# shubhamchandak94/Spring

Hardware: AMD Instinct MI355X
Metric: Mreads/s through reorder stage (higher is better)
Workload: dtype u64; 1 GPU; 100000000 x 150 bp single-end synthetic reads per GPU (uniform genome 600000000 bp, 25x coverage, 1.0% substitutions, 50% reverse-complemented), inputs resident in HBM as .dna records; reads_per_gpu=100000000, read_len=150, chains=65536, num_thr=8, parallelism=single GPU, unmatched=13958636, singletons=12720853, rounds=1984, chain_groups=2

## Files before the change

### include/spring_reorder.h

```cpp
#ifndef SPRING_REORDER_H_
#define SPRING_REORDER_H_

#include <stddef.h>
#include <stdint.h>

#ifdef __cplusplus
extern "C" {
#endif

#define SPRING_REORDER_E_ARG (-1)
#define SPRING_REORDER_E_IO (-2)
#define SPRING_REORDER_E_HIP (-3)
#define SPRING_REORDER_E_STATE (-4)

typedef struct spring_reorder_ctx spring_reorder_ctx;

typedef struct {
  int32_t device;
  uint32_t num_chains;
  int32_t num_thr;
  int32_t collect_stats;
  int32_t time_search;
  int32_t force_literal_update;
  int32_t rounds_per_sync;
// ... 12 lines not shown
  int32_t table_mode;
  int32_t plan0[6];
  int32_t plan1[6];
  int32_t long_min;
  int32_t long_blocks;
  int32_t debug;
  int32_t long_split;
  int32_t entry_flags;
  int32_t out_writers;
  int32_t alternatives;
  int32_t phases;
  int32_t known_absent;
  int32_t sort_prefix_bits;
  int32_t dict_build_mode;
  int32_t strand_filter;
} spring_reorder_opts;

typedef struct {
  uint64_t n_reads, n_matched, n_single, unmatched;
  uint64_t probes, keyok, cands, hits, iterations, rounds, lost;
  uint64_t numkeys[2], dict_numreads[2];
  double ms_unpack, ms_dict, ms_chains, ms_finalize, ms_total;
  double ms_search_kernel;
  uint64_t search_launches;
  uint64_t device_bytes;
  double ms_exchange, ms_resolve_mark;
  uint64_t chains;
  uint64_t deep_pool;
  uint64_t long_searches;
  uint64_t table_minz;
  uint64_t table_marked_lines;
  uint64_t long_splits;
  uint64_t alternatives;
  uint64_t phases;
  double ms_search_busy;
  uint64_t sort_prefix_bits;
  uint64_t sort_repaired_runs;
  uint64_t sort_full_sorts;
  uint64_t sort_long_runs;
  uint64_t sort_list_overflows;
  uint64_t dict_build_path;
  uint64_t strand_filter;
  uint64_t strand_filter_dropped;
} spring_reorder_stats;

void spring_reorder_default_opts(spring_reorder_opts *o);
const char *spring_reorder_last_error(void);
void spring_reorder_trim_pool(void);

int spring_reorder_run(const char *temp_dir, uint32_t max_readlen, int32_t num_thr, int32_t paired_end,
                       uint32_t num_reads_clean_0, uint32_t num_reads_clean_1,
                       const spring_reorder_opts *opts );

int spring_reorder_create(spring_reorder_ctx **ctx, const spring_reorder_opts *opts);
void spring_reorder_destroy(spring_reorder_ctx *ctx);

int spring_reorder_load_dna(spring_reorder_ctx *ctx, const uint8_t *dna, size_t nbytes, uint32_t n,
                            uint32_t max_readlen);

int spring_reorder_load_dna_device(spring_reorder_ctx *ctx, const void *d_dna, size_t nbytes, uint32_t n,
                                   uint32_t max_readlen, int32_t fixed_len);

int spring_reorder_build_dict(spring_reorder_ctx *ctx);

int spring_reorder_run_chains(spring_reorder_ctx *ctx);
int spring_reorder_auto_chains(spring_reorder_ctx *ctx, uint32_t *chains, int32_t *deep);

typedef struct {
  uint32_t num_reads[2], num_reads_clean[2], num_reads_N[2];
  uint32_t max_readlen;
  uint32_t pad;
  double ms_device;
} spring_fastq_info;
int spring_reorder_load_fastq(spring_reorder_ctx *ctx, const uint8_t *fastq_1, size_t nbytes_1, const uint8_t *fastq_2,
                              size_t nbytes_2 , spring_fastq_info *info);
int spring_reorder_fastq_N(spring_reorder_ctx *ctx, int32_t which, uint8_t *n_dna, size_t cap, size_t *nbytes,
                           uint32_t *order_N, uint32_t *count);

// ... 62 lines not shown
```

### spring_amd/_lib.py

```python
import ctypes as C
import os

HERE = os.path.dirname(os.path.abspath(__file__))
LIB_PATH = os.environ.get("SPRING_AMD_LIB") or os.path.join(HERE, "lib", "libspring_reorder_hip.so")

EXPORTS = [
    "spring_reorder_default_opts", "spring_reorder_last_error", "spring_reorder_trim_pool", "spring_reorder_run", "spring_reorder_create",
    "spring_reorder_destroy", "spring_reorder_load_dna", "spring_reorder_load_dna_device",
    "spring_reorder_build_dict", "spring_reorder_run_chains", "spring_reorder_auto_chains", "spring_reorder_finalize",
    "spring_reorder_mg_begin", "spring_reorder_mg_search", "spring_reorder_mg_slice", "spring_reorder_mg_slices",
    "spring_reorder_mg_apply",
    "spring_reorder_mg_end", "spring_reorder_mg_exchange_virtual", "spring_reorder_debug_check_seed_state",
    "spring_mg_rccl_unique_id", "spring_mg_comm_create_rccl", "spring_mg_comm_create_host", "spring_mg_comm_destroy",
    "spring_reorder_mg_run",
    "spring_reorder_get_stats", "spring_reorder_download", "spring_reorder_tid_split", "spring_reorder_emit_dna",
    "spring_reorder_dict_lookup", "spring_reorder_download_reads", "spring_synth_dna_bytes",
    "spring_reorder_load_fastq", "spring_reorder_fastq_N",
    "spring_order_invert_se", "spring_order_invert_pe", "spring_order_correct", "spring_order_pe_encode",
    "spring_fastq_reorder",
    "spring_synth_dna_host", "spring_synth_genome_host", "spring_synth_dna_device", "spring_reorder_load_synth", "spring_reorder_download_dna",
    "spring_encoder_create", "spring_encoder_destroy", "spring_encoder_set_split_tables", "spring_encoder_encode_reorder", "spring_encoder_download",
    "spring_encoder_download_seq_packed", "spring_encoder_get_info", "spring_reorder_encode_run", "spring_encoder_encode_host", "spring_encoder_run",
]

STREAMS_EXPORTS = [
    "spring_streams_create", "spring_streams_destroy", "spring_streams_from_encoder", "spring_streams_from_host",
    "spring_streams_download", "spring_streams_get_info", "spring_streams_run",
]
STREAMS_NUM = 9

DECODE_EXPORTS = [
# ... 13 lines not shown
    "spring_fastq_out_write", "spring_fastq_out_get_info",
]


class Opts(C.Structure):
    _fields_ = [("device", C.c_int32), ("num_chains", C.c_uint32), ("num_thr", C.c_int32),
                ("collect_stats", C.c_int32), ("time_search", C.c_int32), ("force_literal_update", C.c_int32),
                ("rounds_per_sync", C.c_int32), ("long_budget", C.c_int32),
                ("first_shifts", C.c_int32), ("seed_wide", C.c_int32), ("tab_scale", C.c_int32),
                ("search_wpb", C.c_int32), ("dbg_search_lds", C.c_int32), ("dbg_apply_lds", C.c_int32),
                ("fused", C.c_int32), ("deep_bins", C.c_int32),
                ("num_devices", C.c_int32), ("devices", C.c_int32 * 8), ("mg_host_transport", C.c_int32),
                ("table_mode", C.c_int32), ("plan0", C.c_int32 * 6), ("plan1", C.c_int32 * 6), ("long_min", C.c_int32),
                ("long_blocks", C.c_int32), ("debug", C.c_int32), ("long_split", C.c_int32), ("entry_flags", C.c_int32),
                ("out_writers", C.c_int32), ("alternatives", C.c_int32), ("phases", C.c_int32), ("known_absent", C.c_int32),
                ("sort_prefix_bits", C.c_int32), ("dict_build_mode", C.c_int32), ("strand_filter", C.c_int32)]


class FastqInfo(C.Structure):
    _fields_ = [("num_reads", C.c_uint32 * 2), ("num_reads_clean", C.c_uint32 * 2), ("num_reads_N", C.c_uint32 * 2),
                ("max_readlen", C.c_uint32), ("pad", C.c_uint32), ("ms_device", C.c_double)]


class EncoderInfo(C.Structure):
    _fields_ = ([(k, C.c_uint64) for k in ("n_aligned", "n_total", "seq_len", "noise_bytes", "n_noisepos",
                                           "unaligned_bytes", "len_unaligned", "num_contigs")]
                + [(k, C.c_uint32) for k in ("matched_s", "matched_N", "align_passes", "max_bin")]
                + [("ms_device", C.c_double), ("ms_phase", C.c_double * 8)])

    def asdict(self):
        d = {}
# ... 64 lines not shown


class Stats(C.Structure):
    _fields_ = ([(k, C.c_uint64) for k in ("n_reads", "n_matched", "n_single", "unmatched", "probes", "keyok",
                                          "cands", "hits", "iterations", "rounds", "lost")]
                + [("numkeys", C.c_uint64 * 2), ("dict_numreads", C.c_uint64 * 2)]
                + [(k, C.c_double) for k in ("ms_unpack", "ms_dict", "ms_chains", "ms_finalize", "ms_total",
                                             "ms_search_kernel")]
                + [("search_launches", C.c_uint64), ("device_bytes", C.c_uint64),
                   ("ms_exchange", C.c_double), ("ms_resolve_mark", C.c_double), ("chains", C.c_uint64),
                   ("deep_pool", C.c_uint64), ("long_searches", C.c_uint64),
                   ("table_minz", C.c_uint64), ("table_marked_lines", C.c_uint64), ("long_splits", C.c_uint64), ("alternatives", C.c_uint64), ("phases", C.c_uint64),
                   ("ms_search_busy", C.c_double),
                   ("sort_prefix_bits", C.c_uint64), ("sort_repaired_runs", C.c_uint64), ("sort_full_sorts", C.c_uint64),
                   ("sort_long_runs", C.c_uint64), ("sort_list_overflows", C.c_uint64), ("dict_build_path", C.c_uint64),
                   ("strand_filter", C.c_uint64), ("strand_filter_dropped", C.c_uint64)])

    def asdict(self):
        d = {}
        for k, _ in self._fields_:
            v = getattr(self, k)
            d[k] = list(v) if hasattr(v, "__len__") else v
        return d


MG_ALLGATHER_FN = C.CFUNCTYPE(C.c_int, C.c_void_p, C.c_size_t, C.c_size_t, C.c_size_t, C.c_void_p)

_lib = None


def lib():
# ... 27 lines not shown
                                           C.POINTER(C.c_uint32)]
    L.spring_reorder_debug_check_seed_state.argtypes = [vp, C.c_int32, C.POINTER(C.c_uint64)]
    L.spring_reorder_mg_apply.argtypes = [vp, C.c_int32, C.POINTER(C.c_uint32)]
    L.spring_reorder_mg_end.argtypes = [vp]
    L.spring_reorder_mg_exchange_virtual.argtypes = [C.POINTER(vp), C.c_uint32]
    L.spring_mg_rccl_unique_id.argtypes = [vp]
    L.spring_mg_comm_create_rccl.argtypes = [C.POINTER(vp), C.c_int32, vp, C.c_uint32, C.c_uint32]
    L.spring_mg_comm_create_host.argtypes = [C.POINTER(vp), MG_ALLGATHER_FN, vp, C.c_uint32, C.c_uint32]
    L.spring_mg_comm_destroy.argtypes = [vp]
    L.spring_mg_comm_destroy.restype = None
    L.spring_reorder_mg_run.argtypes = [vp, vp, C.c_uint32]
    L.spring_reorder_get_stats.argtypes = [vp, C.POINTER(Stats)]
    L.spring_reorder_download.argtypes = [vp] + [vp] * 8
    L.spring_reorder_tid_split.argtypes = [vp, vp, vp]
    L.spring_reorder_emit_dna.argtypes = [vp, C.c_int32, u8p, C.c_size_t, C.POINTER(C.c_size_t)]
    L.spring_reorder_dict_lookup.argtypes = [vp, C.c_int32, vp, C.c_uint32, vp, vp, C.c_size_t]
    L.spring_reorder_download_reads.argtypes = [vp, vp, vp]
    L.spring_reorder_load_fastq.argtypes = [vp, vp, C.c_size_t, vp, C.c_size_t, C.POINTER(FastqInfo)]
    L.spring_reorder_fastq_N.argtypes = [vp, C.c_int32, vp, C.c_size_t, C.POINTER(C.c_size_t), vp, C.POINTER(C.c_uint32)]
    L.spring_order_invert_se.argtypes = [vp, C.c_uint32, vp, C.POINTER(C.c_double)]
    L.spring_order_invert_pe.argtypes = [vp, C.c_uint32, vp, C.POINTER(C.c_double)]
    L.spring_fastq_reorder.argtypes = [u8p, C.c_size_t, vp, C.c_uint32, u8p, C.c_size_t, C.POINTER(C.c_size_t),
                                       C.POINTER(C.c_double)]
    L.spring_order_pe_encode.argtypes = [vp, C.c_uint32, vp, C.POINTER(C.c_double)]
    L.spring_order_correct.argtypes = [vp, C.c_uint64, vp, C.c_uint32, C.c_uint32, C.POINTER(C.c_double)]
    L.spring_synth_dna_bytes.restype = C.c_size_t
    L.spring_synth_dna_bytes.argtypes = [C.c_uint32, C.c_uint32]
    L.spring_synth_dna_host.argtypes = [u8p, C.c_uint32, C.c_uint32, C.c_uint64, C.c_uint64, C.c_uint32]
    L.spring_synth_genome_host.argtypes = [u8p, C.c_uint64, C.c_uint64, C.c_uint32]
    L.spring_synth_dna_device.argtypes = [vp, C.c_uint32, C.c_uint32, C.c_uint64, C.c_uint64, C.c_uint32]
# ... 80 lines not shown
```

### spring_amd/csrc/dict_build.h

```cpp
#ifndef SPRING_DICT_BUILD_H_
#define SPRING_DICT_BUILD_H_

#include "reorder_device.h"

namespace sr {

bool launch_unpack_keys(hipStream_t st, const uint8_t *dna, uint32_t n, int L, int W, int S, uint32_t rec_fixed,
                        uint64_t *reads, uint16_t *lens, uint32_t *bad_len, int dstart0, int dend0, int dstart1, int dend1,
                        uint64_t *keys0, uint32_t *vals0, uint64_t *keys1, uint32_t *vals1);

constexpr int TAB_WRITE_LG = 10;
inline int tab_write_lg(int bshift) { return 64 - bshift < TAB_WRITE_LG ? 64 - bshift : TAB_WRITE_LG; }
inline uint32_t tab_write_blocks(int bshift) { return (uint32_t)(1ull << (64 - bshift - tab_write_lg(bshift))); }
void launch_tab_partition(hipStream_t st, const uint64_t *h0, uint32_t nk0, const uint64_t *h1, uint32_t nk1, int bshift,
                          uint32_t *part);
constexpr uint32_t TAB_OVF_SLOTS = 8;
void launch_tab_write(hipStream_t st, const uint64_t *h0, uint32_t nk0, const uint64_t *h1, uint32_t nk1,
                      const uint32_t *part, DictBuild d0, DictBuild d1, uint4 *fpt, int bshift, uint32_t *ovf,
                      uint32_t *ovf_blk, uint32_t *ovf_cnt);
void launch_tab_overflow_blocks(hipStream_t st, const uint64_t *h0, uint32_t nk0, const uint64_t *h1, DictBuild d0,
                                DictBuild d1, uint32_t *fpt, int bshift, const uint32_t *ovf_blk, const uint32_t *ovf_cnt);
void launch_tab_overflow_pairs(hipStream_t st, const uint64_t *h0, uint32_t nk0, const uint64_t *h1, DictBuild d0,
                               DictBuild d1, uint32_t *fpt, int bshift, const uint32_t *ovf, uint32_t novf);

constexpr uint32_t PRES_DROP_CTRS = 1024;
void launch_pres_insert(hipStream_t st, const uint64_t *h0, uint32_t nk0, const uint64_t *h1, uint32_t nk1, int wl, uint32_t *pres,
                        int lgb, uint32_t *drops);

}

#endif
```

### spring_amd/csrc/dict_build.hip

```cpp
#include <hip/hip_runtime.h>

#include "dict_build.h"
#include "strand_filter.h"

namespace sr {

__device__ __forceinline__ uint64_t db_mix64(uint64_t x) {
  x ^= x >> 33; x *= 0xff51afd7ed558ccdull; x ^= x >> 33; x *= 0xc4ceb9fe1a85ec53ull; x ^= x >> 33;
  return x;
}
__device__ __forceinline__ uint64_t db_unmix64(uint64_t x) {
  x ^= x >> 33; x *= 0x9cb4b2f8129337dbull; x ^= x >> 33; x *= 0x4f74430c22a54005ull; x ^= x >> 33;
  return x;
}
__device__ __forceinline__ uint32_t db_fp30_of(uint64_t h) {
  const uint32_t f = (uint32_t)h & 0x3fffffffu;
  return f == 0u ? 1u : f == 0x3fffffffu ? 0x3ffffffeu : f;
}

__global__ __launch_bounds__(256) void k_unpack_fixed_keys(const uint8_t *__restrict__ dna, uint32_t n, int L, int W, int lgS,
                                                           uint32_t rec, uint64_t *__restrict__ reads,
                                                           uint16_t *__restrict__ lens, uint32_t *__restrict__ bad_len,
                                                           int dstart0, int klen0, int dstart1, int klen1,
                                                           uint64_t *__restrict__ keys0, uint32_t *__restrict__ vals0,
// ... 285 lines not shown
        placed = true;
      }
    }
    if (!placed) atomicAdd(&s_drop, 1u);
  }
  __syncthreads();
  if (threadIdx.x == 0 && s_drop) atomicAdd(drops + (blockIdx.x & (PRES_DROP_CTRS - 1u)), s_drop);
}
void launch_pres_insert(hipStream_t st, const uint64_t *h0, uint32_t nk0, const uint64_t *h1, uint32_t nk1, int wl, uint32_t *pres,
                        int lgb, uint32_t *drops) {
  const uint64_t nt = (uint64_t)nk0 + nk1;
  if (!nt) return;
  hipLaunchKernelGGL(k_pres_insert, dim3((unsigned)((nt + 255) / 256)), dim3(256), 0, st, h0, nk0, h1, nk1, wl, pres, lgb, drops);
}

}
```

### spring_amd/csrc/reorder_pipeline.cpp

```cpp
#include <hip/hip_runtime.h>
#include <dlfcn.h>

#include <algorithm>
#include <system_error>
#include <thread>
#include <memory>
#include <atomic>
#include <chrono>
#include <cstdarg>
#include <cstdio>
#include <cstdlib>
#include <cstring>
#include <map>
#include <mutex>
#include <new>
#include <stdexcept>
#include <string>
#include <unordered_map>
#include <vector>
#include <zlib.h>

#include "reorder_device.h"
#include "dict_build.h"
#include "reorder_internal.h"
// ... 310 lines not shown
    for (auto &kv : p.free_blocks) { (void)hipFree(kv.second); p.sizes.erase(kv.second); }
    p.free_blocks.clear();
    p.cached = 0;
  }
}

int spring_reorder_create(spring_reorder_ctx **out, const spring_reorder_opts *opts) {
  if (!out) return fail(SPRING_REORDER_E_ARG, "ctx is NULL");
  spring_reorder_opts o;
  if (opts) o = *opts; else spring_reorder_default_opts(&o);
  if (o.num_thr <= 0) return fail(SPRING_REORDER_E_ARG, "num_thr must be >= 1");
  if (o.sort_prefix_bits < 0 || o.sort_prefix_bits > 64)
    return fail(SPRING_REORDER_E_ARG, "sort_prefix_bits: 0 (library's choice) or 1 .. 64 bits of the key hash (64 = the full sort)");
  if (o.dict_build_mode < 0 || o.dict_build_mode > 1)
    return fail(SPRING_REORDER_E_ARG, "dict_build_mode: 0 (library's choice) or 1 (key pass, memset, merge and insert passes)");
  if (o.strand_filter < -1 || o.strand_filter > 32)
    return fail(SPRING_REORDER_E_ARG, "strand_filter: 0 (library's choice), -1 (off) or 1 .. 32 (on, at most 2^n buckets)");
  int ndev = 0;
  HIPCHK(hipGetDeviceCount(&ndev));
  if (ndev <= 0) return fail(SPRING_REORDER_E_HIP, "no HIP device");
  int dev = o.device;
  if (dev < 0) HIPCHK(hipGetDevice(&dev));
  if (dev >= ndev) return fail(SPRING_REORDER_E_ARG, "device %d out of range (%d devices)", dev, ndev);
  HIPCHK(hipSetDevice(dev));
  spring_reorder_ctx *ctx = new spring_reorder_ctx();
  ctx->o = o;
  ctx->dev = dev;
  memset(&ctx->P, 0, sizeof(ctx->P));
  memset(&ctx->stats, 0, sizeof(ctx->stats));
  HIPCHK(hipStreamCreateWithFlags(&ctx->st, hipStreamNonBlocking));
// ... 808 lines not shown
  }
  const uint64_t nk0 = ctx->dict[0].numkeys, nk1 = ctx->dict[1].numkeys, nm = nk0 + nk1;
  const int tab_scale = ctx->o.tab_scale > 0 ? ctx->o.tab_scale : 2;
  const uint64_t nb = std::max<uint64_t>(8, pow2ceil(std::max<uint64_t>(2, (nm * 10 + 15) / 16)) * (uint64_t)pow2ceil(tab_scale));
  ctx->bshift = 64;
  for (uint64_t v = nb; v > 1; v >>= 1) ctx->bshift--;
  ctx->minz = (ctx->dict[0].end - ctx->dict[0].start + 1 == MINZ_WL && ctx->L <= 192 && ctx->o.table_mode == 2) ? 1 : 0;
  ctx->lshift = 32 - (64 - ctx->bshift - 2);
  if (ctx->lshift < 1) return fail(SPRING_REORDER_E_ARG, "build_dict: table too large for minimizer addressing");
  ctx->stats.table_minz = ctx->minz; ctx->stats.table_marked_lines = 0;
  DMALLOC(ctx->fpt, nb * 32);
  const bool one_pass = nm && !ctx->minz && ctx->o.dict_build_mode != 1;
  if (!one_pass) HIPCHK(hipMemsetAsync(ctx->fpt, 0, nb * 32, st));
  uint32_t *const tab_words = reinterpret_cast<uint32_t *>(ctx->fpt);
  DBG_T("alloc+memset tab");
  if (one_pass) {
    if (nm >= 0xffffffffull) return fail(SPRING_REORDER_E_ARG, "build_dict: %llu keys exceed the 32-bit index space of the table build", (unsigned long long)nm);
    ctx->stats.dict_build_path |= 2;
    ctx->marked_lines = 0;
    DictBuild db[2];
    for (int l = 0; l < 2; l++) {
      DictDev &d = ctx->dict[l];
      db[l].ustart = ustart[l]; db[l].ucount = ucount[l]; db[l].ids = d.ids; db[l].urec = d.urec;
      db[l].deep = d.deep; db[l].ndeep = d.d_ndeep;
    }
    uint32_t *d_part = nullptr, *d_ovf = nullptr, *d_ovf_blk = nullptr, *d_ovf_cnt = nullptr, novf = 0;
    const size_t nblk = tab_write_blocks(ctx->bshift);
    DMALLOC(d_part, 2 * (nblk + 1) * 4);
    DMALLOC(d_ovf_blk, nblk * TAB_OVF_SLOTS * 4);
    DMALLOC(d_ovf_cnt, nblk * 4);
    DMALLOC(d_ovf, ((size_t)nm + 1) * 4);
    HIPCHK(hipMemsetAsync(d_ovf, 0, 4, st));
    launch_tab_partition(st, uhash[0], (uint32_t)nk0, uhash[1], (uint32_t)nk1, ctx->bshift, d_part);
    launch_tab_write(st, uhash[0], (uint32_t)nk0, uhash[1], (uint32_t)nk1, d_part, db[0], db[1], ctx->fpt, ctx->bshift, d_ovf,
                     d_ovf_blk, d_ovf_cnt);
    launch_tab_overflow_blocks(st, uhash[0], (uint32_t)nk0, uhash[1], db[0], db[1], tab_words, ctx->bshift, d_ovf_blk, d_ovf_cnt);
    HIPCHK(hipGetLastError());
    HIPCHK(hipMemcpyAsync(&novf, d_ovf, 4, hipMemcpyDeviceToHost, st));
    uint32_t nd[2][3] = {{0, 0, 0}, {0, 0, 0}};
    for (int l = 0; l < 2; l++)
      HIPCHK(hipMemcpyAsync(nd[l], ctx->dict[l].d_ndeep, 12, hipMemcpyDeviceToHost, st));
    HIPCHK(hipStreamSynchronize(st));
    DBG_T("table write");
    launch_tab_overflow_pairs(st, uhash[0], (uint32_t)nk0, uhash[1], db[0], db[1], tab_words, ctx->bshift, d_ovf, novf);
    HIPCHK(hipGetLastError());
    for (int l = 0; l < 2; l++) { ctx->dict[l].ndeep = nd[l][0]; ctx->dict[l].big_reads = nd[l][1]; ctx->dict[l].mid_reads = nd[l][2]; }
    if (dbg) {
      fprintf(stderr, "[dict] %u of %llu pairs past the %u overflow slots of their workgroup\n", novf, (unsigned long long)nm, TAB_OVF_SLOTS);
      fprintf(stderr, "[dict] reads %u + %u, keys %u + %u, bins >= %u: %u + %u, reads in bins >= %u: %u + %u, >= %u: %u + %u\n",
              ctx->dict[0].numreads, ctx->dict[1].numreads, ctx->dict[0].numkeys, ctx->dict[1].numkeys, DEEP_BIN, nd[0][0], nd[1][0],
              MID_BIN, nd[0][2], nd[1][2], BIG_BIN, nd[0][1], nd[1][1]);
    }
// ... 46 lines not shown
      DMALLOC(tp_in, nm * 8); DMALLOC(tp_out, nm * 8);
      launch_minz_prepare(st, h_in, v_in, nm, db[0], db[1], ctx->lshift, bk_in, tp_in);
      DBG_T("minz prepare");
      const unsigned end_bit = (unsigned)(64 - ctx->bshift);
      size_t tb = 0;
      HIPCHK(sort_pairs_u32_u64(st, nullptr, tb, bk_in, bk_out, tp_in, tp_out, nm, end_bit));
      DMALLOC(d_tmp2, tb);
      HIPCHK(sort_pairs_u32_u64(st, d_tmp2, tb, bk_in, bk_out, tp_in, tp_out, nm, end_bit));
      DBG_T("minz sort");
      DMALLOC(d_marked, 16);
      HIPCHK(hipMemsetAsync(d_marked, 0, 4, st));
      launch_tab_insert_minz(st, bk_out, tp_out, nm, tab_words, ctx->bshift, d_marked);
      HIPCHK(hipMemcpyAsync(&ctx->marked_lines, d_marked, 4, hipMemcpyDeviceToHost, st));
    }
    HIPCHK(hipGetLastError());
    uint32_t nd[2][3] = {{0, 0, 0}, {0, 0, 0}};
    for (int l = 0; l < 2; l++)
      HIPCHK(hipMemcpyAsync(nd[l], ctx->dict[l].d_ndeep, 12, hipMemcpyDeviceToHost, st));
    HIPCHK(hipStreamSynchronize(st));
    for (int l = 0; l < 2; l++) { ctx->dict[l].ndeep = nd[l][0]; ctx->dict[l].big_reads = nd[l][1]; ctx->dict[l].mid_reads = nd[l][2]; }
    if (dbg) fprintf(stderr, "[dict] reads %u + %u, keys %u + %u, bins >= %u: %u + %u, reads in bins >= %u: %u + %u, >= %u: %u + %u\n",
                     ctx->dict[0].numreads, ctx->dict[1].numreads, ctx->dict[0].numkeys, ctx->dict[1].numkeys, DEEP_BIN, nd[0][0], nd[1][0],
                     MID_BIN, nd[0][2], nd[1][2], BIG_BIN, nd[0][1], nd[1][1]);
    ctx->stats.table_marked_lines = ctx->marked_lines;
    DBG_T("insert");
    ctx->dfree(mv0); ctx->dfree(mh); ctx->dfree(mv); ctx->dfree(d_tmp);
    ctx->dfree(bk_in); ctx->dfree(bk_out); ctx->dfree(tp_in); ctx->dfree(tp_out); ctx->dfree(d_tmp2); ctx->dfree(d_marked); ctx->dfree(d_ovf);
  }
  ctx->pres = nullptr; ctx->pres_lgb = 0;
  ctx->stats.strand_filter = 0; ctx->stats.strand_filter_dropped = 0;
  int lgb = 0;
  if (nm && nm < 0xffffffffull && strand_filter_wanted(ctx)) {
    while (lgb < 32 && (1ull << lgb) < nm) lgb++;
    if (ctx->o.strand_filter > 0) lgb = std::min(lgb, ctx->o.strand_filter);
    if (ctx->dmalloc((void **)&ctx->pres, (size_t)16 << lgb)) {
      (void)hipGetLastError();
      ctx->pres = nullptr;
      if (dbg) fprintf(stderr, "[dict] presence table: no room for 2^%d buckets, running without\n", lgb);
    }
  }
  if (ctx->pres) {
    uint32_t *d_drops = nullptr;
    std::vector<uint32_t> h_drops(PRES_DROP_CTRS);
    DMALLOC(d_drops, PRES_DROP_CTRS * 4);
    HIPCHK(hipMemsetAsync(ctx->pres, 0, (size_t)16 << lgb, st));
    HIPCHK(hipMemsetAsync(d_drops, 0, PRES_DROP_CTRS * 4, st));
    launch_pres_insert(st, uhash[0], (uint32_t)nk0, uhash[1], (uint32_t)nk1, ctx->dict[0].end - ctx->dict[0].start + 1,
                       reinterpret_cast<uint32_t *>(ctx->pres), lgb, d_drops);
    HIPCHK(hipGetLastError());
    HIPCHK(hipMemcpyAsync(h_drops.data(), d_drops, PRES_DROP_CTRS * 4, hipMemcpyDeviceToHost, st));
    HIPCHK(hipStreamSynchronize(st));
    for (uint32_t v : h_drops) ctx->stats.strand_filter_dropped += v;
    ctx->pres_lgb = lgb;
    ctx->dfree(d_drops);
    if (dbg) fprintf(stderr, "[dict] presence table: 2^%d buckets, %llu of %llu keys dropped\n", lgb,
                     (unsigned long long)ctx->stats.strand_filter_dropped, (unsigned long long)nm);
    DBG_T("presence table");
  }
  for (int l = 0; l < 2; l++) { ctx->dfree(uhash[l]); ctx->dfree(ustart[l]); ctx->dfree(ucount[l]); }
  DBG_T("free temps");
  HIPCHK(hipEventRecord(ctx->ev[3], st));
  ctx->stage = ST_DICT;
  return 0;
}

int spring_reorder_dict_lookup(spring_reorder_ctx *ctx, int32_t which, const uint64_t *keys, uint32_t nkeys,
                               uint32_t *bin_size, uint32_t *bin_ids, size_t ids_cap) {
  if (!ctx || ctx->stage < ST_DICT) return fail(SPRING_REORDER_E_STATE, "dict_lookup: build_dict first");
  if (which < 0 || which > 1) return fail(SPRING_REORDER_E_ARG, "which must be 0 or 1");
  HIPCHK(hipSetDevice(ctx->dev));
  DictDev &d = ctx->dict[which];
  uint64_t *dk = nullptr;
  uint32_t *ds = nullptr, *dc = nullptr;
  DMALLOC(dk, (size_t)nkeys * 8);
  DMALLOC(ds, (size_t)nkeys * 4);
  DMALLOC(dc, (size_t)nkeys * 4);
  std::vector<uint32_t> hs(nkeys), hc(nkeys), hids(d.numreads);
// ... 1370 lines not shown
```

### spring_amd/csrc/strand_filter.h

```cpp
#ifndef SPRING_STRAND_FILTER_H_
#define SPRING_STRAND_FILTER_H_

#include <stdint.h>

#if defined(__HIPCC__) || defined(__CUDACC__)
#define SF_FN __host__ __device__ inline
#else
#define SF_FN inline
#endif

namespace sf {

SF_FN uint64_t mix64(uint64_t x) {
  x ^= x >> 33; x *= 0xff51afd7ed558ccdull; x ^= x >> 33; x *= 0xc4ceb9fe1a85ec53ull; x ^= x >> 33;
  return x;
}
SF_FN uint64_t brev64(uint64_t x) {
  x = ((x >> 1) & 0x5555555555555555ull) | ((x & 0x5555555555555555ull) << 1);
  x = ((x >> 2) & 0x3333333333333333ull) | ((x & 0x3333333333333333ull) << 2);
  x = ((x >> 4) & 0x0f0f0f0f0f0f0f0full) | ((x & 0x0f0f0f0f0f0f0f0full) << 4);
  x = ((x >> 8) & 0x00ff00ff00ff00ffull) | ((x & 0x00ff00ff00ff00ffull) << 8);
  x = ((x >> 16) & 0x0000ffff0000ffffull) | ((x & 0x0000ffff0000ffffull) << 16);
  return (x >> 32) | (x << 32);
}
// ... 22 lines not shown
  return r < w ? r : w;
}
SF_FN uint32_t flags_of_key(uint64_t w, int wl, int l) {
  uint32_t f;
  (void)canon_and_flags(w, wl, l, f);
  return f;
}
SF_FN uint32_t absent_of(uint32_t s0, uint32_t s1, uint32_t s2, uint32_t s3, uint32_t fp) {
  const uint32_t f0 = (s0 >> 4) == fp ? s0 : 0u, f1 = (s1 >> 4) == fp ? s1 : 0u, f2 = (s2 >> 4) == fp ? s2 : 0u,
                 f3 = (s3 >> 4) == fp ? s3 : 0u;
  const uint32_t hit = f0 | f1 | f2 | f3;
  return s3 != 0u ? 0u : ~hit & 15u;
}
SF_FN uint32_t to_window_frame(uint32_t a, bool swapped) { return swapped ? ((a >> 2) | (a << 2)) & 15u : a; }

}

#endif
```

### spring_amd/reorder.py

```python
import ctypes as C
from dataclasses import dataclass

import numpy as np

from . import _lib


class ReorderError(RuntimeError):
    """Raised where the reference throws std::runtime_error (call_template_functions.cpp:60)."""


@dataclass
class ReorderOpts:
    device: int = -1
    num_chains: int = 0
    num_thr: int = 1
    collect_stats: bool = False
    time_search: bool = False
    force_literal_update: bool = False
    rounds_per_sync: int = 0
    first_shifts: int = 0
    seed_wide: int = 0
    tab_scale: int = 0
    search_wpb: int = 0
# ... 7 lines not shown
    plan0: tuple = ()
    plan1: tuple = ()
    long_min: int = 0
    long_blocks: int = 0
    entry_flags: int = 0
    long_split: int = 0
    debug: bool = False
    out_writers: int = 0
    alternatives: int = 0
    table_mode: int = 0
    phases: int = 0
    known_absent: int = 0
    sort_prefix_bits: int = 0
    dict_build_mode: int = 0
    strand_filter: int = 0

    def to_c(self):
        o = _lib.Opts()
        _lib.lib().spring_reorder_default_opts(C.byref(o))
        o.device, o.num_chains, o.num_thr = self.device, self.num_chains, self.num_thr
        o.collect_stats, o.time_search = int(self.collect_stats), int(self.time_search)
        o.force_literal_update, o.rounds_per_sync = int(self.force_literal_update), self.rounds_per_sync
        o.first_shifts, o.seed_wide, o.tab_scale = self.first_shifts, self.seed_wide, self.tab_scale
        o.search_wpb, o.dbg_search_lds, o.dbg_apply_lds = self.search_wpb, self.dbg_search_lds, self.dbg_apply_lds
        o.fused, o.deep_bins = self.fused, self.deep_bins
        o.long_budget = self.long_budget
        if len(self.devices) > 8:
            raise ValueError("at most 8 devices")
        o.table_mode = self.table_mode
        for i, v in enumerate(tuple(self.plan0)[:6]):
            o.plan0[i] = int(v)
        for i, v in enumerate(tuple(self.plan1)[:6]):
            o.plan1[i] = int(v)
        o.long_min, o.long_blocks, o.debug = self.long_min, self.long_blocks, int(self.debug)
        o.long_split, o.entry_flags = self.long_split, self.entry_flags
        o.out_writers = self.out_writers
        o.alternatives = self.alternatives
        o.phases = self.phases
        o.known_absent = self.known_absent
        o.sort_prefix_bits = self.sort_prefix_bits
        o.dict_build_mode = self.dict_build_mode
        o.strand_filter = self.strand_filter
        o.num_devices = len(self.devices)
        for i, d in enumerate(self.devices):
            o.devices[i] = d
        o.mg_host_transport = int(self.mg_host_transport)
        return o


def _chk(rc):
    if rc != 0:
        raise ReorderError("%s (code %d)" % (_lib.lib().spring_reorder_last_error().decode(), rc))


class ReorderStage:

    def __init__(self, opts: ReorderOpts = None):
# ... 104 lines not shown
    def emit_dna(self, tid: int) -> bytes:
        nb = C.c_size_t()
        _chk(self._L.spring_reorder_emit_dna(self._h, tid, None, 0, C.byref(nb)))
        buf = np.zeros(max(nb.value, 1), np.uint8)
        _chk(self._L.spring_reorder_emit_dna(self._h, tid, buf.ctypes.data, nb.value, C.byref(nb)))
        return buf[:nb.value].tobytes()

    def dict_lookup(self, which, keys):
        keys = np.ascontiguousarray(keys, dtype=np.uint64)
        sizes = np.zeros(max(len(keys), 1), np.uint32)
        ids = np.zeros(max(self.n, 1) * 2, np.uint32)
        _chk(self._L.spring_reorder_dict_lookup(self._h, which, keys.ctypes.data, len(keys), sizes.ctypes.data,
                                                ids.ctypes.data, len(ids)))
        return sizes[:len(keys)], ids

    def download_reads(self):
        W = (2 * self.max_readlen - 1) // 64 + 1
        limbs = np.zeros((max(self.n, 1), W), np.uint64)
        ln = np.zeros(max(self.n, 1), np.uint16)
        _chk(self._L.spring_reorder_download_reads(self._h, limbs.ctypes.data, ln.ctypes.data))
        return limbs[:self.n], ln[:self.n]

    def download_dna(self) -> bytes:
        nb = self._L.spring_synth_dna_bytes(self.n, self.max_readlen)
        buf = np.zeros(max(nb, 1), np.uint8)
        _chk(self._L.spring_reorder_download_dna(self._h, buf.ctypes.data, nb))
        p = 0
        for _ in range(self.n):
            p += 2 + ((int(buf[p]) | (int(buf[p + 1]) << 8)) + 3) // 4
        return buf[:p].tobytes()
# ... 45 lines not shown
```

Baseline: 362.9 Mreads/s.

## Build presence table by streaming sorted key ranges through LDS-resident blocks

Replaces the global-atomic insert pass for the strand-filter presence table with a blocked build. Keys whose reverse complement is canonical are first compacted into a side list and radix-sorted by bucket prefix. Each workgroup then binary-searches its slice of the already-sorted hash arrays and assembles one table block in LDS with shared atomics before writing it out. This removes the full-table memset and the scattered global atomics and drops one stream synchronize. In exchange it adds a compaction kernel, a rocprim sort, a partition kernel and extra scratch memory, and it falls back to the old pass when allocation fails.

```diff
diff --git a/include/spring_reorder.h b/include/spring_reorder.h
--- a/include/spring_reorder.h
+++ b/include/spring_reorder.h
@@ -50,6 +50,7 @@
   int32_t sort_prefix_bits;
   int32_t dict_build_mode;
   int32_t strand_filter;
+  int32_t pres_build;
 } spring_reorder_opts;
 
 typedef struct {
@@ -78,6 +79,7 @@
   uint64_t dict_build_path;
   uint64_t strand_filter;
   uint64_t strand_filter_dropped;
+  uint64_t pres_build;
 } spring_reorder_stats;
 
 void spring_reorder_default_opts(spring_reorder_opts *o);
@@ -98,6 +100,8 @@
                                    uint32_t max_readlen, int32_t fixed_len);
 
 int spring_reorder_build_dict(spring_reorder_ctx *ctx);
+
+int spring_reorder_pres_table(spring_reorder_ctx *ctx, uint32_t *out, size_t cap_words, int32_t *lgb);
 
 int spring_reorder_run_chains(spring_reorder_ctx *ctx);
 int spring_reorder_auto_chains(spring_reorder_ctx *ctx, uint32_t *chains, int32_t *deep);
diff --git a/spring_amd/_lib.py b/spring_amd/_lib.py
--- a/spring_amd/_lib.py
+++ b/spring_amd/_lib.py
@@ -14,7 +14,7 @@
     "spring_mg_rccl_unique_id", "spring_mg_comm_create_rccl", "spring_mg_comm_create_host", "spring_mg_comm_destroy",
     "spring_reorder_mg_run",
     "spring_reorder_get_stats", "spring_reorder_download", "spring_reorder_tid_split", "spring_reorder_emit_dna",
-    "spring_reorder_dict_lookup", "spring_reorder_download_reads", "spring_synth_dna_bytes",
+    "spring_reorder_dict_lookup", "spring_reorder_pres_table", "spring_reorder_download_reads", "spring_synth_dna_bytes",
     "spring_reorder_load_fastq", "spring_reorder_fastq_N",
     "spring_order_invert_se", "spring_order_invert_pe", "spring_order_correct", "spring_order_pe_encode",
     "spring_fastq_reorder",
@@ -58,7 +58,8 @@
                 ("table_mode", C.c_int32), ("plan0", C.c_int32 * 6), ("plan1", C.c_int32 * 6), ("long_min", C.c_int32),
                 ("long_blocks", C.c_int32), ("debug", C.c_int32), ("long_split", C.c_int32), ("entry_flags", C.c_int32),
                 ("out_writers", C.c_int32), ("alternatives", C.c_int32), ("phases", C.c_int32), ("known_absent", C.c_int32),
-                ("sort_prefix_bits", C.c_int32), ("dict_build_mode", C.c_int32), ("strand_filter", C.c_int32)]
+                ("sort_prefix_bits", C.c_int32), ("dict_build_mode", C.c_int32), ("strand_filter", C.c_int32),
+                ("pres_build", C.c_int32)]
 
 
 class FastqInfo(C.Structure):
@@ -153,7 +154,7 @@
                    ("ms_search_busy", C.c_double),
                    ("sort_prefix_bits", C.c_uint64), ("sort_repaired_runs", C.c_uint64), ("sort_full_sorts", C.c_uint64),
                    ("sort_long_runs", C.c_uint64), ("sort_list_overflows", C.c_uint64), ("dict_build_path", C.c_uint64),
-                   ("strand_filter", C.c_uint64), ("strand_filter_dropped", C.c_uint64)])
+                   ("strand_filter", C.c_uint64), ("strand_filter_dropped", C.c_uint64), ("pres_build", C.c_uint64)])
 
     def asdict(self):
         d = {}
@@ -211,6 +212,7 @@
     L.spring_reorder_download.argtypes = [vp] + [vp] * 8
     L.spring_reorder_tid_split.argtypes = [vp, vp, vp]
     L.spring_reorder_emit_dna.argtypes = [vp, C.c_int32, u8p, C.c_size_t, C.POINTER(C.c_size_t)]
+    L.spring_reorder_pres_table.argtypes = [vp, vp, C.c_size_t, C.POINTER(C.c_int32)]
     L.spring_reorder_dict_lookup.argtypes = [vp, C.c_int32, vp, C.c_uint32, vp, vp, C.c_size_t]
     L.spring_reorder_download_reads.argtypes = [vp, vp, vp]
     L.spring_reorder_load_fastq.argtypes = [vp, vp, C.c_size_t, vp, C.c_size_t, C.POINTER(FastqInfo)]
diff --git a/spring_amd/csrc/dict_build.h b/spring_amd/csrc/dict_build.h
--- a/spring_amd/csrc/dict_build.h
+++ b/spring_amd/csrc/dict_build.h
@@ -27,6 +27,15 @@
 void launch_pres_insert(hipStream_t st, const uint64_t *h0, uint32_t nk0, const uint64_t *h1, uint32_t nk1, int wl, uint32_t *pres,
                         int lgb, uint32_t *drops);
 
+constexpr int PRES_WRITE_LG = 12;
+inline int pres_write_lg(int lgb) { return lgb < PRES_WRITE_LG ? lgb : PRES_WRITE_LG; }
+inline uint32_t pres_write_blocks(int lgb) { return 1u << (lgb - pres_write_lg(lgb)); }
+void launch_pres_swapped(hipStream_t st, const uint64_t *h0, uint32_t nk0, const uint64_t *h1, uint32_t nk1, int wl, uint64_t *ent,
+                         uint32_t *n_ent);
+hipError_t pres_sort_entries(hipStream_t st, void *tmp, size_t &tmp_bytes, const uint64_t *in, uint64_t *out, uint32_t n, int lgb);
+void launch_pres_write(hipStream_t st, const uint64_t *h0, uint32_t nk0, const uint64_t *h1, uint32_t nk1, const uint64_t *ent,
+                       uint32_t nsw, int wl, uint32_t *part, uint4 *pres, int lgb, uint32_t *drops);
+
 }
 
 #endif
diff --git a/spring_amd/csrc/dict_build.hip b/spring_amd/csrc/dict_build.hip
--- a/spring_amd/csrc/dict_build.hip
+++ b/spring_amd/csrc/dict_build.hip
@@ -1,4 +1,8 @@
 #include <hip/hip_runtime.h>
+
+#include <cstring>
+
+#include <rocprim/rocprim.hpp>
 
 #include "dict_build.h"
 #include "strand_filter.h"
@@ -323,4 +327,120 @@
   hipLaunchKernelGGL(k_pres_insert, dim3((unsigned)((nt + 255) / 256)), dim3(256), 0, st, h0, nk0, h1, nk1, wl, pres, lgb, drops);
 }
 
-}
+constexpr uint32_t PRES_SWAP_KEYS = 1024;
+__global__ __launch_bounds__(256) void k_pres_swapped(const uint64_t *__restrict__ h0, uint32_t nk0, const uint64_t *__restrict__ h1,
+                                                      uint32_t nk1, int wl, uint64_t *__restrict__ ent, uint32_t *__restrict__ n_ent) {
+  __shared__ uint64_t s_ent[PRES_SWAP_KEYS];
+  __shared__ uint32_t s_n, s_base;
+  if (threadIdx.x == 0) s_n = 0u;
+  __syncthreads();
+  const uint64_t nt = (uint64_t)nk0 + nk1, base = (uint64_t)blockIdx.x * PRES_SWAP_KEYS;
+  for (uint32_t j = 0; j < PRES_SWAP_KEYS / 256u; j++) {
+    const uint64_t t = base + j * 256u + threadIdx.x;
+    if (t >= nt) break;
+    const int l = t >= nk0 ? 1 : 0;
+    const uint64_t key = db_unmix64(l ? h1[t - nk0] : h0[t]), r = sf::rc_window(key, wl);
+    if (r < key) s_ent[atomicAdd(&s_n, 1u)] = sf::pack_entry(sf::mix64(r), l);
+  }
+  __syncthreads();
+  const uint32_t n = s_n;
+  if (threadIdx.x == 0 && n) s_base = atomicAdd(n_ent, n);
+  __syncthreads();
+  if (n) {
+    uint64_t *__restrict__ out = ent + s_base;
+    for (uint32_t k = threadIdx.x; k < n; k += 256u) out[k] = s_ent[k];
+  }
+}
+
+__global__ void k_pres_partition(const uint64_t *__restrict__ h0, uint32_t nk0, const uint64_t *__restrict__ h1, uint32_t nk1,
+                                 const uint64_t *__restrict__ ent, uint32_t nsw, int lgb, int lg_blk, uint32_t nblk,
+                                 uint32_t *__restrict__ part) {
+  const uint64_t t = (uint64_t)blockIdx.x * blockDim.x + threadIdx.x, per = (uint64_t)nblk + 1;
+  if (t >= 3ull * per) return;
+  const uint32_t a = (uint32_t)(t / per), j = (uint32_t)(t % per);
+  const uint64_t *__restrict__ h = a == 0 ? h0 : a == 1 ? h1 : ent;
+  const uint32_t nk = a == 0 ? nk0 : a == 1 ? nk1 : nsw;
+  uint32_t lo = 0, hi = nk;
+  if (j == nblk) {
+    lo = nk;
+  } else {
+    while (lo < hi) {
+      const uint32_t mid = lo + (hi - lo) / 2;
+      if (sf::block_of(h[mid], lgb, lg_blk) < j) lo = mid + 1; else hi = mid;
+    }
+  }
+  part[t] = lo;
+}
+
+constexpr uint32_t PRES_WRITE_THREADS = 512;
+__global__ __launch_bounds__(PRES_WRITE_THREADS) void k_pres_write(const uint64_t *__restrict__ h0, const uint64_t *__restrict__ h1,
+                                                                   const uint64_t *__restrict__ ent,
+                                                                   const uint32_t *__restrict__ part, uint32_t nblk, int wl,
+                                                                   uint4 *__restrict__ pres, int lgb, int lg_blk,
+                                                                   uint32_t *__restrict__ drops) {
+  __shared__ uint4 img4[1u << PRES_WRITE_LG];
+  uint32_t *img = reinterpret_cast<uint32_t *>(img4);
+  const uint32_t nbk = sf::block_buckets(lgb, lg_blk), bmask = nbk - 1u, blk = blockIdx.x;
+  for (uint32_t k = threadIdx.x; k < nbk; k += PRES_WRITE_THREADS) img4[k] = make_uint4(0u, 0u, 0u, 0u);
+  __syncthreads();
+  uint32_t ndrop = 0;
+  auto enter = [&](uint64_t hc, uint32_t flags) {
+    const uint32_t fp = sf::fp_of(hc), word = (fp << 4) | flags;
+    uint32_t *bk = img + 4u * (sf::bucket_of(hc, lgb) & bmask);
+    for (int sl = 0; sl < 4; sl++) {
+      const uint32_t old = atomicCAS(bk + sl, 0u, word);
+      if (old == 0u) return;
+      if ((old >> 4) == fp) {
+        if ((old & flags) != flags) atomicOr(bk + sl, flags);
+        return;
+      }
+    }
+    ndrop++;
+  };
+  const uint64_t per = (uint64_t)nblk + 1;
+  for (int l = 0; l < 2; l++) {
+    const uint64_t *__restrict__ h = l ? h1 : h0;
+    const uint64_t e = part[l * per + blk + 1];
+    for (uint64_t i = (uint64_t)part[l * per + blk] + threadIdx.x; i < e; i += PRES_WRITE_THREADS) {
+      const uint64_t hh = h[i], key = db_unmix64(hh);
+      uint32_t flags;
+      if (sf::canon_and_flags(key, wl, l, flags) != key) continue;
+      enter(hh, flags);
+    }
+  }
+  {
+    const uint64_t e = part[2 * per + blk + 1];
+    for (uint64_t i = (uint64_t)part[2 * per + blk] + threadIdx.x; i < e; i += PRES_WRITE_THREADS) {
+      const uint64_t x = ent[i];
+      enter(x, 4u << sf::entry_dict(x));
+    }
+  }
+  __syncthreads();
+  uint4 *__restrict__ out = pres + (uint64_t)blk * nbk;
+  for (uint32_t k = threadIdx.x; k < nbk; k += PRES_WRITE_THREADS) out[k] = img4[k];
+  if (ndrop) atomicAdd(drops + (blk & (PRES_DROP_CTRS - 1u)), ndrop);
+}
+
+void launch_pres_swapped(hipStream_t st, const uint64_t *h0, uint32_t nk0, const uint64_t *h1, uint32_t nk1, int wl, uint64_t *ent,
+                         uint32_t *n_ent) {
+  const uint64_t nt = (uint64_t)nk0 + nk1;
+  if (!nt) return;
+  hipLaunchKernelGGL(k_pres_swapped, dim3((unsigned)((nt + PRES_SWAP_KEYS - 1) / PRES_SWAP_KEYS)), dim3(256), 0, st, h0, nk0, h1,
+                     nk1, wl, ent, n_ent);
+}
+hipError_t pres_sort_entries(hipStream_t st, void *tmp, size_t &tmp_bytes, const uint64_t *in, uint64_t *out, uint32_t n, int lgb) {
+  const unsigned begin_bit = (unsigned)(64 - lgb + pres_write_lg(lgb));
+  return rocprim::radix_sort_keys<rocprim::radix_sort_config<rocprim::default_config, rocprim::default_config, rocprim::default_config, 0>>(
+      tmp, tmp_bytes, in, out, (size_t)n, begin_bit, 64u, st);
+}
+void launch_pres_write(hipStream_t st, const uint64_t *h0, uint32_t nk0, const uint64_t *h1, uint32_t nk1, const uint64_t *ent,
+                       uint32_t nsw, int wl, uint32_t *part, uint4 *pres, int lgb, uint32_t *drops) {
+  const int lg_blk = pres_write_lg(lgb);
+  const uint32_t nblk = sf::blocks_of(lgb, lg_blk);
+  const uint64_t nt = 3ull * ((uint64_t)nblk + 1);
+  hipLaunchKernelGGL(k_pres_partition, dim3((unsigned)((nt + 255) / 256)), dim3(256), 0, st, h0, nk0, h1, nk1, ent, nsw, lgb, lg_blk,
+                     nblk, part);
+  hipLaunchKernelGGL(k_pres_write, dim3(nblk), dim3(PRES_WRITE_THREADS), 0, st, h0, h1, ent, part, nblk, wl, pres, lgb, lg_blk, drops);
+}
+
+}
diff --git a/spring_amd/csrc/reorder_pipeline.cpp b/spring_amd/csrc/reorder_pipeline.cpp
--- a/spring_amd/csrc/reorder_pipeline.cpp
+++ b/spring_amd/csrc/reorder_pipeline.cpp
@@ -348,6 +348,8 @@
     return fail(SPRING_REORDER_E_ARG, "sort_prefix_bits: 0 (library's choice) or 1 .. 64 bits of the key hash (64 = the full sort)");
   if (o.dict_build_mode < 0 || o.dict_build_mode > 1)
     return fail(SPRING_REORDER_E_ARG, "dict_build_mode: 0 (library's choice) or 1 (key pass, memset, merge and insert passes)");
+  if (o.pres_build < 0 || o.pres_build > 2)
+    return fail(SPRING_REORDER_E_ARG, "pres_build: 0 (library's choice), 1 (insert pass) or 2 (streamed build)");
   if (o.strand_filter < -1 || o.strand_filter > 32)
     return fail(SPRING_REORDER_E_ARG, "strand_filter: 0 (library's choice), -1 (off) or 1 .. 32 (on, at most 2^n buckets)");
   int ndev = 0;
@@ -1186,6 +1188,31 @@
   if (!one_pass) HIPCHK(hipMemsetAsync(ctx->fpt, 0, nb * 32, st));
   uint32_t *const tab_words = reinterpret_cast<uint32_t *>(ctx->fpt);
   DBG_T("alloc+memset tab");
+  const bool pres_wanted = nm && nm < 0xffffffffull && strand_filter_wanted(ctx);
+  int lgb = 0;
+  if (pres_wanted) {
+    while (lgb < 32 && (1ull << lgb) < nm) lgb++;
+    if (ctx->o.strand_filter > 0) lgb = std::min(lgb, ctx->o.strand_filter);
+  }
+  bool pres_stream = pres_wanted && ctx->o.pres_build != 1 &&
+                     (ctx->o.pres_build == 2 || nm / pres_write_blocks(lgb) <= (1ull << 20));
+  uint64_t *d_ent = nullptr;
+  uint32_t *d_nent = nullptr, nsw = 0;
+  if (pres_stream && (ctx->dmalloc((void **)&d_ent, (size_t)nm * 8) || ctx->dmalloc((void **)&d_nent, 16))) {
+    (void)hipGetLastError();
+    ctx->dfree(d_ent); ctx->dfree(d_nent); d_ent = nullptr; d_nent = nullptr;
+    pres_stream = false;
+    if (dbg) fprintf(stderr, "[dict] presence table: no room for the streamed build's entries, insert pass\n");
+  }
+  const int pres_wl = ctx->dict[0].end - ctx->dict[0].start + 1;
+  auto pres_swapped_pass = [&]() -> int {
+    if (!pres_stream) return 0;
+    HIPCHK(hipMemsetAsync(d_nent, 0, 4, st));
+    launch_pres_swapped(st, uhash[0], (uint32_t)nk0, uhash[1], (uint32_t)nk1, pres_wl, d_ent, d_nent);
+    HIPCHK(hipGetLastError());
+    HIPCHK(hipMemcpyAsync(&nsw, d_nent, 4, hipMemcpyDeviceToHost, st));
+    return 0;
+  };
   if (one_pass) {
     if (nm >= 0xffffffffull) return fail(SPRING_REORDER_E_ARG, "build_dict: %llu keys exceed the 32-bit index space of the table build", (unsigned long long)nm);
     ctx->stats.dict_build_path |= 2;
@@ -1208,6 +1235,7 @@
                      d_ovf_blk, d_ovf_cnt);
     launch_tab_overflow_blocks(st, uhash[0], (uint32_t)nk0, uhash[1], db[0], db[1], tab_words, ctx->bshift, d_ovf_blk, d_ovf_cnt);
     HIPCHK(hipGetLastError());
+    if (int r = pres_swapped_pass()) return r;
     HIPCHK(hipMemcpyAsync(&novf, d_ovf, 4, hipMemcpyDeviceToHost, st));
     uint32_t nd[2][3] = {{0, 0, 0}, {0, 0, 0}};
     for (int l = 0; l < 2; l++)
@@ -1284,6 +1312,7 @@
       HIPCHK(hipMemcpyAsync(&ctx->marked_lines, d_marked, 4, hipMemcpyDeviceToHost, st));
     }
     HIPCHK(hipGetLastError());
+    if (int r = pres_swapped_pass()) return r;
     uint32_t nd[2][3] = {{0, 0, 0}, {0, 0, 0}};
     for (int l = 0; l < 2; l++)
       HIPCHK(hipMemcpyAsync(nd[l], ctx->dict[l].d_ndeep, 12, hipMemcpyDeviceToHost, st));
@@ -1298,11 +1327,12 @@
     ctx->dfree(bk_in); ctx->dfree(bk_out); ctx->dfree(tp_in); ctx->dfree(tp_out); ctx->dfree(d_tmp2); ctx->dfree(d_marked); ctx->dfree(d_ovf);
   }
   ctx->pres = nullptr; ctx->pres_lgb = 0;
-  ctx->stats.strand_filter = 0; ctx->stats.strand_filter_dropped = 0;
-  int lgb = 0;
-  if (nm && nm < 0xffffffffull && strand_filter_wanted(ctx)) {
-    while (lgb < 32 && (1ull << lgb) < nm) lgb++;
-    if (ctx->o.strand_filter > 0) lgb = std::min(lgb, ctx->o.strand_filter);
+  ctx->stats.strand_filter = 0; ctx->stats.strand_filter_dropped = 0; ctx->stats.pres_build = 0;
+  for (int l = 0; l < 2; l++) {
+    ctx->dfree(ustart[l]); ctx->dfree(ucount[l]);
+    ustart[l] = nullptr; ucount[l] = nullptr;
+  }
+  if (pres_wanted) {
     if (ctx->dmalloc((void **)&ctx->pres, (size_t)16 << lgb)) {
       (void)hipGetLastError();
       ctx->pres = nullptr;
@@ -1310,27 +1340,69 @@
     }
   }
   if (ctx->pres) {
-    uint32_t *d_drops = nullptr;
+    uint32_t *d_drops = nullptr, *d_ppart = nullptr;
+    uint64_t *d_ent2 = nullptr, *sorted = d_ent;
+    void *d_stmp = nullptr;
+    size_t stmp_bytes = 0;
     std::vector<uint32_t> h_drops(PRES_DROP_CTRS);
     DMALLOC(d_drops, PRES_DROP_CTRS * 4);
-    HIPCHK(hipMemsetAsync(ctx->pres, 0, (size_t)16 << lgb, st));
     HIPCHK(hipMemsetAsync(d_drops, 0, PRES_DROP_CTRS * 4, st));
-    launch_pres_insert(st, uhash[0], (uint32_t)nk0, uhash[1], (uint32_t)nk1, ctx->dict[0].end - ctx->dict[0].start + 1,
-                       reinterpret_cast<uint32_t *>(ctx->pres), lgb, d_drops);
+    const uint32_t pblk = pres_write_blocks(lgb);
+    const bool need_sort = pres_stream && pblk > 1 && nsw > 1;
+    if (pres_stream) {
+      bool ok = ctx->dmalloc((void **)&d_ppart, 3 * ((size_t)pblk + 1) * 4) == 0;
+      if (ok && need_sort) {
+        ok = ctx->dmalloc((void **)&d_ent2, (size_t)nsw * 8) == 0 &&
+             pres_sort_entries(st, nullptr, stmp_bytes, d_ent, d_ent2, nsw, lgb) == hipSuccess &&
+             ctx->dmalloc(&d_stmp, stmp_bytes) == 0;
+      }
+      if (!ok) {
+        (void)hipGetLastError();
+        pres_stream = false;
+        if (dbg) fprintf(stderr, "[dict] presence table: no room for the streamed build's scratch, insert pass\n");
+      }
+    }
+    if (pres_stream) {
+      if (need_sort) {
+        HIPCHK(pres_sort_entries(st, d_stmp, stmp_bytes, d_ent, d_ent2, nsw, lgb));
+        sorted = d_ent2;
+      }
+      launch_pres_write(st, uhash[0], (uint32_t)nk0, uhash[1], (uint32_t)nk1, sorted, nsw, pres_wl, d_ppart, ctx->pres, lgb, d_drops);
+      ctx->stats.pres_build = 2;
+    } else {
+      HIPCHK(hipMemsetAsync(ctx->pres, 0, (size_t)16 << lgb, st));
+      launch_pres_insert(st, uhash[0], (uint32_t)nk0, uhash[1], (uint32_t)nk1, pres_wl, reinterpret_cast<uint32_t *>(ctx->pres), lgb,
+                         d_drops);
+      ctx->stats.pres_build = 1;
+    }
     HIPCHK(hipGetLastError());
     HIPCHK(hipMemcpyAsync(h_drops.data(), d_drops, PRES_DROP_CTRS * 4, hipMemcpyDeviceToHost, st));
-    HIPCHK(hipStreamSynchronize(st));
+    ctx->dfree(d_ent); ctx->dfree(d_ent2); ctx->dfree(d_stmp); ctx->dfree(d_ppart); d_ent = nullptr;
+    ctx->dfree(d_drops);
     for (uint32_t v : h_drops) ctx->stats.strand_filter_dropped += v;
     ctx->pres_lgb = lgb;
-    ctx->dfree(d_drops);
-    if (dbg) fprintf(stderr, "[dict] presence table: 2^%d buckets, %llu of %llu keys dropped\n", lgb,
-                     (unsigned long long)ctx->stats.strand_filter_dropped, (unsigned long long)nm);
+    if (dbg) fprintf(stderr, "[dict] presence table: 2^%d buckets, %s, %u of %llu keys as sorted entries, %llu dropped\n", lgb,
+                     ctx->stats.pres_build == 2 ? "streamed" : "insert pass", nsw, (unsigned long long)nm,
+                     (unsigned long long)ctx->stats.strand_filter_dropped);
     DBG_T("presence table");
   }
+  ctx->dfree(d_ent); ctx->dfree(d_nent);
   for (int l = 0; l < 2; l++) { ctx->dfree(uhash[l]); ctx->dfree(ustart[l]); ctx->dfree(ucount[l]); }
   DBG_T("free temps");
   HIPCHK(hipEventRecord(ctx->ev[3], st));
   ctx->stage = ST_DICT;
+  return 0;
+}
+
+int spring_reorder_pres_table(spring_reorder_ctx *ctx, uint32_t *out, size_t cap_words, int32_t *lgb) {
+  if (!ctx || ctx->stage < ST_DICT) return fail(SPRING_REORDER_E_STATE, "pres_table: build_dict first");
+  const size_t nw = ctx->pres ? (size_t)4 << ctx->pres_lgb : 0;
+  if (lgb) *lgb = ctx->pres ? ctx->pres_lgb : -1;
+  if (!out || !nw) return 0;
+  if (cap_words < nw) return fail(SPRING_REORDER_E_ARG, "pres_table: room for %zu words, the table has %zu", cap_words, nw);
+  HIPCHK(hipSetDevice(ctx->dev));
+  HIPCHK(hipMemcpyAsync(out, ctx->pres, nw * 4, hipMemcpyDeviceToHost, ctx->st));
+  HIPCHK(hipStreamSynchronize(ctx->st));
   return 0;
 }
 
diff --git a/spring_amd/csrc/strand_filter.h b/spring_amd/csrc/strand_filter.h
--- a/spring_amd/csrc/strand_filter.h
+++ b/spring_amd/csrc/strand_filter.h
@@ -60,6 +60,12 @@
 }
 SF_FN uint32_t to_window_frame(uint32_t a, bool swapped) { return swapped ? ((a >> 2) | (a << 2)) & 15u : a; }
 
+SF_FN uint64_t pack_entry(uint64_t hc, int l) { return (hc & ~(0xfull << 28)) | ((uint64_t)(l & 1) << 28); }
+SF_FN int entry_dict(uint64_t e) { return (int)((e >> 28) & 1u); }
+SF_FN uint32_t block_of(uint64_t h, int lgb, int lg_blk) { return lgb > lg_blk ? (uint32_t)(h >> (64 - lgb + lg_blk)) : 0u; }
+SF_FN uint32_t blocks_of(int lgb, int lg_blk) { return lgb > lg_blk ? 1u << (lgb - lg_blk) : 1u; }
+SF_FN uint32_t block_buckets(int lgb, int lg_blk) { return 1u << (lgb < lg_blk ? lgb : lg_blk); }
+
 }
 
 #endif
diff --git a/spring_amd/reorder.py b/spring_amd/reorder.py
--- a/spring_amd/reorder.py
+++ b/spring_amd/reorder.py
@@ -45,6 +45,7 @@
     sort_prefix_bits: int = 0
     dict_build_mode: int = 0
     strand_filter: int = 0
+    pres_build: int = 0
 
     def to_c(self):
         o = _lib.Opts()
@@ -72,6 +73,7 @@
         o.sort_prefix_bits = self.sort_prefix_bits
         o.dict_build_mode = self.dict_build_mode
         o.strand_filter = self.strand_filter
+        o.pres_build = self.pres_build
         o.num_devices = len(self.devices)
         for i, d in enumerate(self.devices):
             o.devices[i] = d
@@ -206,6 +208,15 @@
                                                 ids.ctypes.data, len(ids)))
         return sizes[:len(keys)], ids
 
+    def presence_table(self):
+        lgb = C.c_int32(-1)
+        _chk(self._L.spring_reorder_pres_table(self._h, None, 0, C.byref(lgb)))
+        if lgb.value < 0:
+            return None, -1
+        out = np.zeros(4 << lgb.value, np.uint32)
+        _chk(self._L.spring_reorder_pres_table(self._h, out.ctypes.data, out.size, C.byref(lgb)))
+        return out.reshape(-1, 4), lgb.value
+
     def download_reads(self):
         W = (2 * self.max_readlen - 1) // 64 + 1
         limbs = np.zeros((max(self.n, 1), W), np.uint64)
```

Measured after the change: 366.1 Mreads/s (median of 6 runs). About the same (+0.9%).
